# k-sheridan/mantis

Hardware: AMD Instinct MI355X
Metric: poses/sec + p50 per-frame latency, 1280x720 4-cam batch (higher is better)
Workload: dtype f64; 1 GPU; config3: 4-cam 1280x720 rig, shared map, full mantis3 path per camera + joint rig Gauss-Newton; cams_per_rig=4, contexts_per_gpu=6, landmarks=720, parallelism=rig-data-parallel x1

## Files before the change

### mantis_amd/csrc/api.hip

```cpp
#include <hip/hip_runtime.h>
#ifndef MK_FC_THREADS
#define MK_FC_THREADS 256
#endif

#include <algorithm>
#include <atomic>
#include <cfloat>
#include <chrono>
#include <cmath>
#include <cstdio>
#include <cstdlib>
#include <cstring>
#include <mutex>
#include <sstream>
#include <string>
#include <thread>
#include <vector>

#include <rccl/rccl.h>

#include "kernels.hip"

using namespace mk;

// ... 865 lines not shown
    if ((st = gauss_offsets(c, n, sh)) != MANTIS_OK) return st;
    gauss.t.join();
    if ((st = run_score(c, n, ng)) != MANTIS_OK) return st;
    if ((st = results_d2h()) != MANTIS_OK) return st;
  }
  if (sh) HIP_OK(hipMemcpyAsync(c->h_sh_flags, c->d_sh_flags, sizeof(int32_t) * ng, hipMemcpyDeviceToHost, c->s));
  HIP_OK(wait_stream(c, n));
  finish_profile(c);
  const int per = c->cfg.particles * c->cfg.iterations * 6;
  int used = 0;
  if (sh)
    for (int f = 0; f < ng; f++) used += c->h_sh_flags[f] ? 1 : 0;
  for (int f = 0; f < n; f++) {
    if (!sh && c->h_st[f].reaches_pf) used++;
    if (c->h_st[f].overflow) {
      std::ostringstream os;
      os << "frame " << f << ": workspace capacity exceeded (flags " << c->h_st[f].overflow << ", borders "
         << c->h_st[f].n_borders << ", points " << c->h_st[f].n_points << ", raw quads " << c->h_st[f].n_raw_quads
         << ")";
      c->err = os.str();
      c->h_res[f].status = MANTIS_ERR_CAPACITY;
    }
  }
  if (const char* fs = getenv("MANTIS_FRAME_STATS")) {
    if (FILE* fp = fopen(fs, "a")) {
      for (int f = 0; f < n; f++)
        fprintf(fp, "%d %d %d %d %d %d %d\n", c->h_st[f].n_runs, c->h_st[f].n_borders, c->h_st[f].n_points,
                c->h_st[f].trace_steps_max, c->h_st[f].trace_steps_sum, c->h_st[f].n_chunks, c->h_st[f].trace_ticks);
      fclose(fp);
    }
  }
  if (used * per != *c->h_gtotal) { c->err = "internal: gaussian stream accounting mismatch"; return MANTIS_ERR_DEVICE; }
  c->frame_rng.resize(n);
  if (sh) {
    std::vector<int> upto(ng + 1, 0);
    for (int f = 0; f < ng; f++) upto[f + 1] = upto[f] + (c->h_sh_flags[f] ? 1 : 0);
    for (int f = 0; f < n; f++) c->frame_rng[f] = c->h_states[upto[sh->gidx[f] + 1]];
  } else {
    int k = 0;
    for (int f = 0; f < n; f++) {
      if (c->h_st[f].reaches_pf) k++;
      c->frame_rng[f] = c->h_states[k];
    }
  }
  c->rng_state = c->h_states[used];
  return MANTIS_OK;
}

template <class T>
mantis_status dalloc(Ctx* c, T** p, size_t count) {
  if (hipMalloc((void**)p, sizeof(T) * std::max<size_t>(count, 1)) != hipSuccess) {
    c->err = "hipMalloc failed";
    return MANTIS_ERR_OOM;
  }
  return MANTIS_OK;
}
struct DevScratch {
  Ctx* c;
  std::vector<void*> p;
  explicit DevScratch(Ctx* ctx) : c(ctx) {}
  template <class T>
  bool get(T** q, size_t count) {
    *q = nullptr;
    if (dalloc(c, q, count)) return true;
    p.push_back((void*)*q);
    return false;
  }
  ~DevScratch() {
    if (!p.empty()) (void)hipStreamSynchronize(c->s);
    for (void* q : p) (void)hipFree(q);
  }
};
template <class T>
mantis_status halloc(Ctx* c, T** p, size_t count) {
  if (hipHostMalloc((void**)p, sizeof(T) * std::max<size_t>(count, 1), hipHostMallocDefault) != hipSuccess) {
    c->err = "hipHostMalloc failed";
    return MANTIS_ERR_OOM;
  }
  return MANTIS_OK;
}

std::vector<double> gather_tbc(const mantis_image* cams, int n) {
  std::vector<double> T(16 * (size_t)n);
  for (int i = 0; i < n; i++) std::memcpy(&T[16 * (size_t)i], cams[i].T_base_cam, sizeof(double) * 16);
  return T;
}

thread_local std::string g_create_err;

}

extern "C" {

int32_t mantis_abi_version(void) { return MANTIS_ABI_VERSION; }

void mantis_default_config(mantis_config* cfg) {
  std::memset(cfg, 0, sizeof(*cfg));
  cfg->struct_size = sizeof(mantis_config);
  cfg->device = 0;
  cfg->max_cams = 16;
  cfg->max_width = 1280;
  cfg->max_height = 720;
  cfg->rng_seed = 1;
  cfg->canny_low = 50;
  cfg->polygon_epsilon = 10;
  cfg->search_radius_multiplier = 0.1;
  cfg->grid_spacing = 0.32;
  cfg->particles = 50;
  cfg->iterations = 10;
  cfg->gn_enable = 0;
  cfg->gn_iterations = 10;
  cfg->max_quads = kMaxQuads;
  cfg->max_contour_points = 262144;
  cfg->quad_gn_iterations = 0;
  cfg->rig_weighting = 0;
}

mantis_status mantis_create(const mantis_config* cfg_in, void** out_ctx) {
  if (!out_ctx) return MANTIS_ERR_ARG;
  *out_ctx = nullptr;
  mantis_config cfg;
  mantis_default_config(&cfg);
  if (cfg_in) {
    if (cfg_in->struct_size != (int32_t)sizeof(mantis_config)) {
      g_create_err = "mantis_config.struct_size mismatch";
      return MANTIS_ERR_ARG;
    }
    cfg = *cfg_in;
  }
  if (cfg.max_quads == 0) cfg.max_quads = kMaxQuads;
  if ((int64_t)cfg.particles * cfg.iterations * 6 * (cfg.max_cams > 0 ? cfg.max_cams : 1) > INT32_MAX) {
    g_create_err = "particles x iterations x 6 x max_cams exceeds 2^31 gaussians per batch";
    return MANTIS_ERR_ARG;
  }
  if (cfg.particles < 1 || cfg.particles > 96 || cfg.iterations < 0 || cfg.iterations > 1000 || cfg.max_cams < 1 ||
      cfg.max_width < 3 || cfg.max_height < 3 || cfg.gn_iterations < 0 || cfg.gn_iterations > 10 ||
      cfg.quad_gn_iterations < 0 || cfg.quad_gn_iterations > 20 || cfg.rig_weighting < 0 || cfg.rig_weighting > 1) {
    g_create_err = "invalid config (particles 1..96, iterations 0..1000, gn_iterations 0..10, "
                   "quad_gn_iterations 0..20, max_cams >= 1, image >= 3x3)";
    return MANTIS_ERR_ARG;
  }
  if (cfg.max_width > 8190) {
    g_create_err = "max_width: at most 8190 (the hysteresis bands hold a row's worst-case runs in LDS)";
    return MANTIS_ERR_ARG;
  }
  if (cfg.max_height > 65533) {
    g_create_err = "max_height: at most 65533 (border walks and contour points pack y + 1 in 16 bits)";
    return MANTIS_ERR_ARG;
  }
  if ((int64_t)((cfg.max_height + HB_ROWS - 1) / HB_ROWS) * HB_ROWS * ((cfg.max_width + 1) / 2) >= (1 << 24)) {
    g_create_err = "max_width x max_height: at most 2^25 pixels (hysteresis run ids and their band row share a word)";
    return MANTIS_ERR_ARG;
  }
  if (cfg.max_quads != kMaxQuads) {
    g_create_err = "max_quads: the per-frame quad capacity is fixed at 256 in this build";
    return MANTIS_ERR_ARG;
  }
  int ndev = 0;
  if (hipGetDeviceCount(&ndev) != hipSuccess || ndev <= cfg.device) {
    g_create_err = "no HIP device available (libmantis_amd requires an MI355X / gfx950 GPU)";
    return MANTIS_ERR_DEVICE;
  }
  Ctx* c = new Ctx();
  c->cfg = cfg;
  c->rng_state = cfg.rng_seed ? cfg.rng_seed : 0xffffffffULL;
  if (hipSetDevice(cfg.device) != hipSuccess || hipStreamCreateWithFlags(&c->s, hipStreamNonBlocking) != hipSuccess ||
      hipStreamCreateWithFlags(&c->s_copy, hipStreamNonBlocking) != hipSuccess ||
      hipEventCreateWithFlags(&c->ev_gauss, hipEventDisableTiming) != hipSuccess ||
      hipEventCreateWithFlags(&c->ev_wait, hipEventDisableTiming | hipEventBlockingSync) != hipSuccess) {
    g_create_err = "hipSetDevice/hipStreamCreate failed";
    if (c->s) (void)hipStreamDestroy(c->s);
    if (c->s_copy) (void)hipStreamDestroy(c->s_copy);
    delete c;
    return MANTIS_ERR_DEVICE;
  }
  if (hipDeviceGetAttribute(&c->n_cu, hipDeviceAttributeMultiprocessorCount, cfg.device) != hipSuccess || c->n_cu < 1)
    c->n_cu = 256;
  if (const char* e = std::getenv("MANTIS_RPP_BLOCKS")) c->rpp_blocks = std::atoi(e);
  if (const char* e = std::getenv("MANTIS_OP_ROUNDS")) c->op_rounds = std::max(1, std::min(kOpMaxRounds, std::atoi(e)));
  if (const char* e = std::getenv("MANTIS_OP_SPILL")) c->op_spill = std::max(0, std::min(64, std::atoi(e)));
  if (const char* e = std::getenv("MANTIS_OP_LANES_SMALL")) c->op_lanes_small = std::max(1, std::min(64, std::atoi(e)));
  if (const char* e = std::getenv("MANTIS_OP_ROUNDS_SMALL")) c->op_rounds_small = std::max(1, std::min(kOpMaxRounds, std::atoi(e)));
  if (const char* e = std::getenv("MANTIS_SEG_M")) c->seg_m = std::max(0, std::min(4096, std::atoi(e)));
  if (const char* e = std::getenv("MANTIS_CANNY_STRIP")) c->canny_strip = c->canny_small = std::atoi(e);
  if (const char* e = std::getenv("MANTIS_CANNY_CAT")) c->canny_cat = e[0] != '0';
  if (const char* e = std::getenv("MANTIS_GN_FUSED")) c->gn_fused_all = e[0] != '0';
  if (const char* e = std::getenv("MANTIS_PF_INIT")) c->pf_init = std::max(0, std::min(2, std::atoi(e)));
  if (const char* e = std::getenv("MANTIS_HYST_REC")) c->hyst_rec = e[0] != '0';
  {
    const char* pc = std::getenv("DEBUG_CLR_GRAPH_PACKET_CAPTURE");
    c->use_graphs = pc && pc[0] == '0';
    if (const char* e = std::getenv("MANTIS_GRAPHS")) c->use_graphs = c->use_graphs && e[0] != '0';
  }
  if (const char* e = std::getenv("MANTIS_HYST_EPOCH0")) c->hyst_epoch = std::max(3, std::min(255, std::atoi(e)));
  c->F = cfg.max_cams;
  c->Wmax = cfg.max_width;
  c->Hmax = cfg.max_height;
  c->plane = (size_t)(c->Wmax + 2) * (c->Hmax + 2);
  c->bstride = bits::tiled_words(c->Wmax, c->Hmax);
  c->dstride = (size_t)dbits_wpw(c->Wmax + 2) * (c->Hmax + 2);
  c->pool_cap = cfg.max_contour_points;
  {
    c->trace_lds_max = 160 * 1024 - 512 * 8 - 64;
    c->trace_lds_ok = hipFuncSetAttribute((const void*)k_trace_borders_lds, hipFuncAttributeMaxDynamicSharedMemorySize,
                                          (int)c->trace_lds_max) == hipSuccess;
    const char* so = getenv("MANTIS_SCREEN");
    c->screen_off = so && so[0] == '0';
    const char* e = getenv("MANTIS_TRACE_LDS_FRAMES");
    c->trace_lds_frames = e ? atoi(e) : c->n_cu / 4;
    const char* e2 = getenv("MANTIS_FC_SMALL_FRAMES");
    c->fc_small_frames = e2 ? atoi(e2) : c->n_cu / 4;
    const char* e3 = getenv("MANTIS_PF_SPLIT");
    c->pf_split = !(e3 && e3[0] == '0');
  }
  {
    const size_t ml = bits::tiled_words(c->Wmax, c->Hmax) * 4;
    hipFuncAttributes a1;
    c->pf_mask_lds = 0;
    if (!getenv("MANTIS_PF_MASK_GLOBAL") &&
        hipFuncGetAttributes(&a1, (const void*)k_score_pf<kPfThreads, kPfSplit, true>) == hipSuccess &&
        a1.sharedSizeBytes + ml <= 160 * 1024 &&
        hipFuncSetAttribute((const void*)k_score_pf<kPfThreads, kPfSplit, true>,
                            hipFuncAttributeMaxDynamicSharedMemorySize, (int)ml) == hipSuccess)
      c->pf_mask_lds = ml;
  }
  {
    hipFuncAttributes a;
    if (hipFuncGetAttributes(&a, (const void*)k_hyst_rec) == hipSuccess) {
      const size_t budget = 160 * 1024 - a.sharedSizeBytes;
      if (hipFuncSetAttribute((const void*)k_hyst_rec, hipFuncAttributeMaxDynamicSharedMemorySize, (int)budget) ==
          hipSuccess)
        c->hyst_rec_lds = budget;
    }
  }
  if (hipFuncSetAttribute((const void*)k_hyst_band, hipFuncAttributeMaxDynamicSharedMemorySize,
                          (int)(3 * sizeof(uint32_t) * HB_ROWS * bits::words(c->Wmax))) != hipSuccess) {
    g_create_err = "max_width too large for the hysteresis band kernel";
    (void)hipStreamDestroy(c->s);
    delete c;
    return MANTIS_ERR_ARG;
  }
  c->morph_bh = morph_lds(c->Wmax, MB_BH) <= 160 * 1024 ? MB_BH : MB_BH_NARROW;
  if (const char* e = getenv("MANTIS_MORPH_WALK")) {
    c->morph_walk = std::max(0, atoi(e));
    c->morph_walk_small = std::max(1, c->morph_walk);
  }
  if (const char* e = getenv("MANTIS_MORPH_WALK_SMALL")) c->morph_walk_small = std::max(1, atoi(e));
  if (morph_lds(c->Wmax, c->morph_bh) > 160 * 1024 ||
      hipFuncSetAttribute((const void*)k_morph, hipFuncAttributeMaxDynamicSharedMemorySize,
                          (int)morph_lds(c->Wmax, c->morph_bh)) !=
          hipSuccess) {
    g_create_err = "max_width too large for the morphology band kernel";
    (void)hipStreamDestroy(c->s);
    delete c;
    return MANTIS_ERR_ARG;
  }
  const int F = c->F;
  const int per = cfg.particles * cfg.iterations * 6;
  mantis_status st = MANTIS_OK;
  auto chk = [&](mantis_status s) { if (st == MANTIS_OK) st = s; };
  c->fstride = (c->plane + 3) & ~(size_t)3;
  chk(dalloc(c, &c->d_strong, (size_t)F * c->fstride));
  c->lstride = (c->plane + 1) & ~(size_t)1;
  chk(dalloc(c, &c->d_lroot, (size_t)F * c->lstride));
  chk(dalloc(c, &c->d_edge, c->plane));
  chk(dalloc(c, &c->d_det, c->plane));
  chk(dalloc(c, &c->d_eb, (size_t)F * c->bstride));
  chk(dalloc(c, &c->d_b1, (size_t)F * c->bstride));
  chk(dalloc(c, &c->d_b2, (size_t)F * c->bstride));
  chk(dalloc(c, &c->d_dbits, (size_t)F * c->dstride));
  c->tstride = tbits_words(c->Wmax + 2, c->Hmax + 2);
  chk(dalloc(c, &c->d_tbits, (size_t)F * c->tstride));
  c->rstride = (size_t)c->Hmax + 3 + (c->Hmax + HB_ROWS - 1) / HB_ROWS;
  chk(dalloc(c, &c->d_rowb, (size_t)F * c->rstride));
  chk(dalloc(c, &c->d_mask, c->plane));
  chk(dalloc(c, &c->d_mbits, (size_t)F * c->bstride));
  chk(dalloc(c, &c->d_lab, (size_t)F * c->plane));
  chk(dalloc(c, &c->d_frames, (size_t)F));
  chk(dalloc(c, &c->d_borders, (size_t)F * kMaxBorders));
  chk(dalloc(c, &c->d_bcount, (size_t)F * kMaxBorders));
  chk(dalloc(c, &c->d_boff, (size_t)F * kMaxBorders));
  chk(dalloc(c, &c->d_pool, (size_t)F * 2 * c->pool_cap));
  chk(dalloc(c, &c->d_scratch, (size_t)F * 4 * c->pool_cap));
  chk(dalloc(c, &c->d_quads, (size_t)F * kMaxQuads));
  chk(dalloc(c, &c->d_rpp, (size_t)F * kMaxQuads * 2));
  chk(dalloc(c, &c->d_items, (size_t)F * kMaxQuads * 2));
  chk(dalloc(c, &c->d_refine, (size_t)F * kMaxQuads * 2 * rpp::kCand));
  chk(dalloc(c, &c->d_jobs0, (size_t)F * kMaxQuads * 2));
  chk(dalloc(c, &c->d_jobs1, (size_t)F * kMaxQuads * 2 * rpp::kCand));
  chk(dalloc(c, &c->d_rq, 1));
  {
    const size_t blocks = c->rpp_blocks > 0 ? (size_t)c->rpp_blocks : (size_t)std::max(64, 3 * c->n_cu / 2);
    c->op_cap = (int32_t)(blocks * 256);
    for (int k = 0; k < 2; k++) {
      chk(dalloc(c, &c->d_opool[k], (size_t)kOpFields * c->op_cap));
      chk(dalloc(c, &c->d_ojob[k], (size_t)c->op_cap));
    }
    chk(dalloc(c, &c->d_octl, 2 * 2 * kOpMaxRounds));
  }
  chk(dalloc(c, &c->d_gen, (size_t)F * kMaxHyps));
  chk(dalloc(c, &c->d_hyps, (size_t)F * kMaxHyps));
  chk(dalloc(c, &c->d_st, (size_t)F));
  chk(dalloc(c, &c->d_sst, (size_t)F));
  chk(dalloc(c, &c->d_dbg, (size_t)F));
  chk(dalloc(c, &c->d_res, (size_t)F));
  chk(dalloc(c, &c->d_gauss, (size_t)F * per));
// ... 909 lines not shown
```

### mantis_amd/csrc/kernels.hip

```cpp
#include <hip/hip_runtime.h>

#include <cfloat>
#include <cstdint>
#include <type_traits>

#include "mk_bits.h"
#include "mk_contour.h"
#include "mk_gn.h"
#include "mk_math.h"
#include "mk_rpp.h"
#include "mk_shard.h"
#include "mk_sort.h"
#include "mk_track.h"
#include "mk_types.h"
#include "synth.h"

namespace mk {

#ifndef MK_DPP_SCAN
#define MK_DPP_SCAN 1
#endif
__device__ inline int wave_incl_scan(int v, int lane) {
#if MK_DPP_SCAN
  (void)lane;
// ... 1975 lines not shown
    if (best > 0) rs_s = bj;
    le_eps = best <= eps;
  }
  if (!le_eps) {
    const int sl_s = pos % count, sl_e = (rs_s + sl_s) % count;
    if (lane == 0) {
      stk[0] = sl_e; stk[1] = sl_s;
      stk[2] = sl_s; stk[3] = sl_e;
    }
    top = 2;
  } else {
    if (lane == 0) { dst[0] = spx; dst[1] = spy; }
    nc = 1;
  }
  while (top > 0) {
    top--;
    int a0 = 0, a1 = 0;
    if (lane == 0) { a0 = stk[2 * top]; a1 = stk[2 * top + 1]; }
    const int sl_s = __shfl(a0, 0), sl_e = __shfl(a1, 0);
    const int epx = PtPacked::x(src[sl_e]), epy = PtPacked::y(src[sl_e]);
    int p0 = sl_s + 1;
    if (p0 >= count) p0 = 0;
    spx = PtPacked::x(src[sl_s]);
    spy = PtPacked::y(src[sl_s]);
    if (p0 != sl_e) {
      const double dx = epx - spx, dy = epy - spy;
      int L = sl_e - p0;
      if (L < 0) L += count;
      double best = 0;
      int bt = 0x7fffffff;
      for (int t = lane; t < L; t += 64) {
        int q = p0 + t;
        if (q >= count) q -= count;
        const uint32_t v = src[q];
        const double dist = fabs((PtPacked::y(v) - spy) * dx - (PtPacked::x(v) - spx) * dy);
        if (dist > best) { best = dist; bt = t; }
      }
      wave_argmax(best, bt);
      if (best > 0) rs_s = (p0 + bt) % count;
      le_eps = best * best <= eps * (dx * dx + dy * dy);
    } else {
      le_eps = true;
    }
    if (le_eps) {
      if (lane == 0) { dst[2 * nc] = spx; dst[2 * nc + 1] = spy; }
      nc++;
      if (max_dp > 0 && nc >= max_dp) return max_dp + 1;
    } else {
      if (top + 2 > cap) return -1;
      if (lane == 0) {
        stk[2 * top] = rs_s; stk[2 * top + 1] = sl_e;
        stk[2 * top + 2] = sl_s; stk[2 * top + 3] = rs_s;
      }
      top += 2;
    }
  }
  int r = 0;
  if (lane == 0) r = approx_cleanup(dst, nc, eps, true);
  return __shfl(r, 0);
}

__device__ inline bool ccomp_before(int pa, int ha, int ka, int pb, int hb, int kb) {
  if (pa != pb) return pa > pb;
  if (ha != hb) return ha < hb;
  return ka > kb;
}

#ifndef MK_LONG_BORDER
#define MK_LONG_BORDER 128
#endif
constexpr int kLongBorder = MK_LONG_BORDER;
static_assert(kLongBorder <= 128, "k_frame_contours' length buckets (count / 4) hold counts up to 128");
constexpr int kMaxLong = 512;

struct RawQuad {
  int32_t c[8];
  int32_t parent, hole, key;
};

constexpr int kTbRows = 34;
__device__ __host__ inline int tb_groups(int Wp) { return ((Wp - 2) >> 4) + 1; }
__device__ __host__ inline size_t tbits_words(int Wp, int Hp) {
  return (size_t)tb_groups(Wp) * kTbRows * (size_t)((Hp + 31) >> 5);
}
__device__ inline uint32_t tb_off(int x, int y, int G) {
  return (uint32_t)(((y >> 5) * G + (x >> 4)) * kTbRows + (y & 31));
}
__global__ __launch_bounds__(256) void k_tile_bits(const uint32_t* __restrict__ dbits, size_t dstride,
                                                   uint32_t* __restrict__ tbits, size_t tstride, int wpw, int Wp,
                                                   int Hp) {
  extern __shared__ uint32_t tl_band[];
  const int f = blockIdx.y, ty = blockIdx.x, t = threadIdx.x;
  const uint32_t* src = dbits + (size_t)f * dstride;
  const int r0 = 32 * ty - 1;
  for (int i = t; i < kTbRows * wpw; i += 256) {
    const int e = i / wpw, r = r0 + e;
    tl_band[i] = r >= 0 && r < Hp ? src[(size_t)r * wpw + (i - e * wpw)] : 0u;
  }
  __syncthreads();
  const int G = tb_groups(Wp);
  uint32_t* dst = tbits + (size_t)f * tstride + (size_t)ty * G * kTbRows;
  for (int o = t; o < G * kTbRows; o += 256) {
    const int g = o / kTbRows, e = o - g * kTbRows;
    const int p = 16 * g - 8, w = p >> 5, sh = p & 31;
    const uint32_t lo = w >= 0 ? tl_band[e * wpw + w] : 0u, hi = w + 1 < wpw ? tl_band[e * wpw + w + 1] : 0u;
    dst[o] = (lo >> sh) | (hi << (32 - sh));
  }
}
struct BitsTiled {
  const uint32_t* __restrict__ b;
  int G;
  __device__ uint32_t operator()(int x, int y) const {
    const uint32_t* p = b + tb_off(x, y, G);
    const int sh = (x & 15) + 7;
    return nb8_from_rows((p[0] >> sh) & 7u, (p[1] >> sh) & 7u, (p[2] >> sh) & 7u);
  }
};

#ifndef MK_WALK_WINDOW
#define MK_WALK_WINDOW 1
#endif
struct Walk {
  uint32_t pos, spos, p1;
  int s, prev_s, n, steps;
  int first;
  uint32_t ck, c0, c1, c2, c3;
};
__device__ inline uint32_t wpos(int x, int y) { return (uint32_t)x | ((uint32_t)y << 16); }
__device__ inline uint32_t wdelta(int s) { return (uint32_t)(fdx(s) + (fdy(s) << 16)); }
template <class NB, class EM>
__device__ inline bool walk_start(const NB& nb, int sx, int sy, bool hole, EM& em, Walk& w) {
  const uint32_t m = nb(sx, sy);
  const int s_end0 = hole ? 0 : 4;
  int s = s_end0;
  do {
    s = (s - 1) & 7;
  } while (!((m >> s) & 1u) && s != s_end0);
  w.n = 0;
  w.steps = 0;
  if (s == s_end0) {
    em(sx - 1, sy - 1);
    w.n = 1;
    return false;
  }
  w.spos = w.pos = wpos(sx, sy);
  w.p1 = wpos(sx + fdx(s), sy + fdy(s));
  w.prev_s = s ^ 4;
  w.s = s;
  w.ck = ~0u;
  return true;
}
constexpr int kSegRows = 512;
constexpr int kSegCap = 65536;
struct SegTab {
  int32_t* rowbase;
  int32_t *border, *pos, *sdir, *next, *cnt, *off;
  int cap;
};
__device__ inline SegTab seg_tab(int32_t* sc, int pool_cap) {
  const long mc = pool_cap / kChunk;
  int32_t* base = sc + 2 * (size_t)pool_cap + 3 * (size_t)mc;
  const long avail = 4L * pool_cap - (2L * pool_cap + 3L * mc) - kSegRows;
  SegTab t;
  t.cap = (int)(avail / 6 < kSegCap ? avail / 6 : kSegCap);
  t.rowbase = base;
  int32_t* q = base + kSegRows;
  t.border = q;
  t.pos = q + t.cap;
  t.sdir = q + 2 * (size_t)t.cap;
  t.next = q + 3 * (size_t)t.cap;
  t.cnt = q + 4 * (size_t)t.cap;
  t.off = q + 5 * (size_t)t.cap;
  return t;
}
constexpr int kSegUnused = -1, kSegAlias = -2, kSegStart = -3, kSegSingle = -4;
__device__ inline int seg_id_at(int x, int y, int side, int M, const int32_t* r, const uint16_t* X,
                                const int32_t* rowbase) {
  const int j0 = r[y];
  const int j = j0 + run_at(X + j0, r[y + 1] - j0, x);
  return rowbase[y / M - 1] + 2 * ((j - j0 - 1) >> 1) + side;
}
__device__ inline bool arc_has(int s, int sn, int d) { return ((d - s - 1) & 7) < ((sn - s - 1) & 7); }
__device__ inline int first_cw(uint32_t m, int d) {
  int s = d;
  do {
    s = (s - 1) & 7;
  } while (!((m >> s) & 1u) && s != d);
  return s;
}
template <class NB>
__device__ inline void seg_begin(const NB& nb, const Border& b, int Wp, uint32_t pos, int sd, Walk& w) {
  const int sx = b.start % Wp, sy = b.start / Wp;
  const int s0 = first_cw(nb(sx, sy), b.hole ? 0 : 4);
  w.spos = wpos(sx, sy);
  w.p1 = wpos(sx + fdx(s0), sy + fdy(s0));
  w.pos = pos;
  w.s = sd;
  w.prev_s = (sd + 4) & 7;
  w.n = 0;
  w.steps = 0;
  w.first = 1;
  w.ck = ~0u;
}
template <class EM>
__device__ inline bool walk_step(const uint32_t* __restrict__ tb, int G, const uint8_t* lut, EM& em, Walk& w,
                                 int M, const int32_t* r, const uint16_t* X, const int32_t* rowbase, int& nx) {
  const int x = (int)(w.pos & 0xffffu), y = (int)(w.pos >> 16);
#if MK_WALK_WINDOW
  const uint32_t tg = (uint32_t)((y >> 5) * G + (x >> 4));
  const int yr = y & 31;
  int d = yr - (int)(w.ck & 31u);
  if ((w.ck >> 5) != tg || (unsigned)d > 1u) {
    const int s0 = fdy(w.s ^ 4) < 0 ? max(yr - 1, 0) : min(yr, 30);
    typedef unsigned int u32x4a __attribute__((ext_vector_type(4), aligned(4)));
    const u32x4a v = *(const __attribute__((address_space(1))) u32x4a*)((const char*)tb + ((tg * kTbRows + s0) << 2));
    w.c0 = v.x; w.c1 = v.y; w.c2 = v.z; w.c3 = v.w;
    w.ck = (tg << 5) | (uint32_t)s0;
    d = yr - s0;
  }
  const uint32_t va = d ? w.c1 : w.c0, vb = d ? w.c2 : w.c1, vc = d ? w.c3 : w.c2;
  const int sh = (x & 15) + 7;
  const uint32_t p9 = ((va >> sh) & 7u) | (((vb >> sh) & 7u) << 3) | (((vc >> sh) & 7u) << 6);
#else
  typedef unsigned int u32x3a __attribute__((ext_vector_type(3), aligned(4)));
  const u32x3a v = *(const __attribute__((address_space(1))) u32x3a*)((const char*)tb + (tb_off(x, y, G) << 2));
  const int sh = (x & 15) + 7;
  const uint32_t p9 = ((v.x >> sh) & 7u) | (((v.y >> sh) & 7u) << 3) | (((v.z >> sh) & 7u) << 6);
#endif
  const int s = lut[(p9 << 3) | w.s];
  if (M > 0 && !w.first && y % M == 0) {
    const bool west = arc_has(w.s, s, 4);
    if (west || arc_has(w.s, s, 0)) {
      nx = seg_id_at(x, y, west ? 0 : 1, M, r, X, rowbase);
      return false;
    }
  }
  w.first = 0;
  if (s != w.prev_s) {
    em(x - 1, y - 1);
    w.n++;
    w.prev_s = s;
  }
  const uint32_t np = w.pos + wdelta(s);
  if (np == w.spos && w.pos == w.p1) {
    nx = -1;
    return false;
  }
  w.pos = np;
  w.s = (s + 4) & 7;
  w.steps++;
  return true;
}

struct BitsRows {
  const uint32_t* b;
  int wpw;
  __device__ uint32_t row3(int x, int y) const {
    const uint32_t* p = b + (size_t)y * wpw + ((x - 1) >> 5);
    const uint64_t v = ((uint64_t)p[1] << 32) | p[0];
    return (uint32_t)(v >> ((x - 1) & 31)) & 7u;
  }
  __device__ uint32_t operator()(int x, int y) const { return nb8_from_rows(row3(x, y - 1), row3(x, y), row3(x, y + 1)); }
};
__global__ __launch_bounds__(256) void k_seg_plan(const uint32_t* __restrict__ dbits, size_t dstride,
                                                  const int32_t* __restrict__ rowb, size_t rstride,
                                                  const uint16_t* __restrict__ rx, int32_t* lab, size_t plane,
                                                  const Border* __restrict__ borders, FrameState* st,
                                                  int32_t* __restrict__ scratch, int pool_cap, int Wp, int Hp,
                                                  int border_cap, int M) {
  __shared__ int32_t rb[kSegRows + 1];
  __shared__ int32_t wsum[4];
  const int f = blockIdx.x, t = threadIdx.x, lane = t & 63, wave = t >> 6;
  const int32_t* r = rowb + (size_t)f * rstride;
  const uint16_t* X = rx + (size_t)f * plane;
  int32_t* L = lab + (size_t)f * plane;
  const int nruns = r[Hp];
  const int32_t* bidx = L + nruns;
  int nb = st[f].n_borders;
  if (nb > border_cap) nb = border_cap;
  SegTab T = seg_tab(scratch + 4 * (size_t)f * pool_cap, pool_cap);
  if (nb > T.cap) {
    if (t == 0) atomicOr(&st[f].overflow, 2);
    nb = T.cap;
  }
  const Border* bs = borders + (size_t)f * border_cap;
  const int nsr = M > 0 ? (Hp - 2) / M : 0;
  bool split = M > 0 && nsr > 0 && nsr <= kSegRows && 2 * (size_t)nruns <= plane;
  static_assert(kSegRows <= 512, "two passes of 256 sampled rows");
  int carry = 0;
  for (int pass = 0; pass < 2; pass++) {
    int v = 0;
    const int k = pass * 256 + t;
    if (split && k < nsr) {
      const int y = (k + 1) * M;
      v = 2 * ((r[y + 1] - r[y] - 1) >> 1);
    }
    const int inc = wave_incl_scan(v, lane);
    if (lane == 63) wsum[wave] = inc;
    __syncthreads();
    int o = carry;
    for (int q = 0; q < wave; q++) o += wsum[q];
    if (k < kSegRows) rb[k] = o + inc - v;
    carry += wsum[0] + wsum[1] + wsum[2] + wsum[3];
    __syncthreads();
  }
  int NC = split ? carry : 0;
  if (NC + nb > T.cap) {
    split = false;
    NC = 0;
  }
  if (t == 0) {
    st[f].seg_nc = NC;
    st[f].seg_m = split ? M : 0;
  }
  for (int k = t; k < nsr && split; k += 256) T.rowbase[k] = rb[k];
  const BitsRows nbh{dbits + (size_t)f * dstride, dbits_wpw(Wp)};
  if (split) {
    for (int k = 0; k < nsr; k++) {
      const int y = (k + 1) * M, j0 = r[y], nfg = (r[y + 1] - j0 - 1) >> 1;
      for (int i = t; i < nfg; i += 256) {
        const int g = j0 + 2 * i + 1;
        const int x0 = X[g], x1 = (int)X[g + 1] - 1;
        const int fr = uf_find_c(L, g);
        const int id = rb[k] + 2 * i;
        {
          const int bg = uf_find_c(L, g - 1);
          const int own = (bg != 0 && uf_find_c(L, bg - 1) == fr) ? bg : fr;
          const uint32_t m = nbh(x0, y);
          const int sd = first_cw(m, 4);
          T.border[id] = bidx[own];
          T.pos[id] = (int32_t)wpos(x0, y);
          T.sdir[id] = sd == 4 ? kSegSingle : sd;
          T.next[id] = -1;
          T.cnt[id] = 0;
        }
        {
          const int bg = uf_find_c(L, g + 1);
          const int own = (bg != 0 && uf_find_c(L, bg - 1) == fr) ? bg : fr;
          const uint32_t m = nbh(x1, y);
          int sd = first_cw(m, 0);
          if (sd == 0) {
            sd = kSegUnused;
          } else if (x1 == x0) {
            const int sw = first_cw(m, 4);
            const uint32_t rr = ((m | (m << 8)) >> (sw + 1)) & 0xffu;
            if (arc_has(sw, (sw + 1 + __builtin_ctz(rr)) & 7, 0)) sd = kSegUnused;
          }
          T.border[id + 1] = bidx[own];
          T.pos[id + 1] = (int32_t)wpos(x1, y);
          T.sdir[id + 1] = sd;
          T.next[id + 1] = -1;
          T.cnt[id + 1] = 0;
        }
      }
    }
  }
  __syncthreads();
  for (int b = t; b < nb; b += 256) {
    const Border bb = bs[b];
    const int sx = bb.start % Wp, sy = bb.start / Wp, id = NC + b;
    T.border[id] = b;
    T.cnt[id] = 0;
    T.pos[id] = (int32_t)wpos(sx, sy);
    if (split && sy % M == 0 && sy <= Hp - 2) {
      T.sdir[id] = kSegAlias;
      int c = seg_id_at(sx, sy, bb.hole ? 1 : 0, M, r, X, rb);
      if (T.sdir[c] == kSegUnused) c--;
      T.next[id] = c;
    } else {
      T.sdir[id] = kSegStart;
      T.next[id] = -1;
    }
  }
}

__global__ __launch_bounds__(256) void k_seg_chain(FrameState* st, int32_t* __restrict__ counts,
                                                   int32_t* __restrict__ scratch, int pool_cap, int border_cap) {
  const int f = blockIdx.x, t = threadIdx.x;
  int nb = st[f].n_borders;
  if (nb > border_cap) nb = border_cap;
  int32_t* sc = scratch + 4 * (size_t)f * pool_cap;
  SegTab T = seg_tab(sc, pool_cap);
  int32_t* cnt = counts + (size_t)f * border_cap;
  for (int b = T.cap + t; b < nb; b += 256) cnt[b] = 0;
  if (nb > T.cap) nb = T.cap;
  const int NC = st[f].seg_nc, NS = NC + nb;
  for (int b = t; b < nb; b += 256) {
    const int start = T.sdir[NC + b] == kSegAlias ? T.next[NC + b] : NC + b;
    int cur = start, acc = 0, k = 0;
    bool bad = false;
    do {
      if (++k > NS || T.border[cur] != b) {
        bad = true;
        break;
      }
      T.off[cur] = acc;
      acc += T.cnt[cur];
      cur = T.next[cur];
    } while (cur >= 0 && cur != start);
    cnt[b] = acc;
    if (bad) atomicOr(&st[f].overflow, 2);
  }
  __syncthreads();
  const int max_chunks = pool_cap / kChunk;
  int nch = st[f].n_chunks;
  if (nch > max_chunks) nch = max_chunks;
  int32_t* owner = sc + 2 * (size_t)pool_cap;
  int32_t* ordv = owner + max_chunks;
  for (int c = t; c < nch; c += 256) {
    const int sg = owner[c];
    owner[c] = T.border[sg];
    ordv[c] += T.off[sg];
  }
}

#ifndef MK_TB_WAVES
#define MK_TB_WAVES 4
#endif
__global__ __launch_bounds__(64 * MK_TB_WAVES) void k_trace_borders(const uint32_t* __restrict__ tbits, size_t tstride,
                                                      const Border* __restrict__ borders, FrameState* st,
                                                      int32_t* __restrict__ scratch, int pool_cap, int Wp,
                                                      int border_cap, const int32_t* __restrict__ rowb,
                                                      size_t rstride, const uint16_t* __restrict__ rx, size_t plane) {
  const uint64_t t_start = wall_clock64();
  __shared__ uint8_t next_lut[512 * 8];
  __shared__ int32_t next_job;
  const int f = blockIdx.x, lane = threadIdx.x & 63;
  build_next_lut(next_lut, threadIdx.x, blockDim.x);
  if (threadIdx.x == 0) next_job = 0;
  __syncthreads();
  int nb = st[f].n_borders;
  if (nb > border_cap) nb = border_cap;
  const uint32_t* B = tbits + (size_t)f * tstride;
  const int wpw = dbits_wpw(Wp);
  const Border* bs = borders + (size_t)f * border_cap;
  int32_t* sc = scratch + 4 * (size_t)f * pool_cap;
  const int max_chunks = pool_cap / kChunk;
  int32_t* chunks = sc;
  int32_t* owner = sc + 2 * (size_t)pool_cap;
  int32_t* ordv = owner + max_chunks;
  int32_t* ccount = ordv + max_chunks;
  const SegTab T = seg_tab(sc, pool_cap);
  if (nb > T.cap) nb = T.cap;
  const int NC = st[f].seg_nc, M = st[f].seg_m, NS = NC + nb;
  const int32_t* r = rowb + (size_t)f * rstride;
  const uint16_t* X = rx + (size_t)f * plane;
  const BitsTiled nbh{B, tb_groups(Wp)};
  int32_t* smax = &st[f].trace_steps_max;
  ChunkEmit em{chunks, owner, ordv, ccount, &st[f].n_chunks, max_chunks, 0, -1, 0, 0, false};
  Walk w;
  int i = -1;
  bool act = false;
  bool exhausted = NS == 0;
  const uint64_t below = (1ull << lane) - 1;
  const auto finish = [&](int nx) {
    T.cnt[i] = w.n;
    T.next[i] = nx;
    em.flush();
    if (em.ovf) atomicOr(&st[f].overflow, 2);
    atomicMax(smax, w.steps);
    atomicAdd(&st[f].trace_steps_sum, w.steps);
  };
  for (;;) {
    const uint64_t idle = __ballot(!act);
    const int nidle = __popcll(idle);
    if (!exhausted && (nidle >= 16 || nidle == 64)) {
      const int leader = __ffsll((unsigned long long)idle) - 1;
      int next = 0;
      if (lane == leader) next = atomicAdd(&next_job, nidle);
      next = __shfl(next, leader);
      if (next + nidle >= NS) exhausted = true;
      if (!act) {
        const int j = next + __popcll(idle & below);
        if (j < NS) {
          const int sd = T.sdir[j];
          if (sd != kSegUnused && sd != kSegAlias) {
            i = j;
            const Border b = bs[T.border[j]];
            em.border = j; em.cur = -1; em.k = 0; em.nch = 0; em.ovf = false;
            if (sd == kSegStart) {
              act = walk_start(nbh, b.start % Wp, b.start / Wp, b.hole != 0, em, w);
              w.first = 0;
              if (!act) finish(-1);
            } else if (sd == kSegSingle) {
              const uint32_t p = (uint32_t)T.pos[j];
              em((int)(p & 0xffffu) - 1, (int)(p >> 16) - 1);
              w.n = 1;
              w.steps = 0;
              finish(-1);
            } else {
              seg_begin(nbh, b, Wp, (uint32_t)T.pos[j], sd, w);
              act = true;
            }
          }
        }
      }
      continue;
    }
    if (nidle == 64) {
      if (exhausted) break;
      continue;
    }
    int nx = -1;
    if (act && !walk_step(nbh.b, nbh.G, next_lut, em, w, M, r, X, T.rowbase, nx)) {
      act = false;
      finish(nx);
    }
  }
  if (lane == 0) atomicMax(&st[f].trace_ticks, (int32_t)(wall_clock64() - t_start));
}

extern __shared__ uint32_t tb_lds[];
struct BitsNBLds {
  int wpw;
  __device__ uint32_t row3(int x, int y) const {
    const int o = y * wpw + ((x - 1) >> 5);
    const uint64_t v = ((uint64_t)tb_lds[o + 1] << 32) | tb_lds[o];
    return (uint32_t)(v >> ((x - 1) & 31)) & 7u;
  }
  __device__ uint32_t operator()(int x, int y) const { return nb8_from_rows(row3(x, y - 1), row3(x, y), row3(x, y + 1)); }
};
template <class NB, class EM>
__device__ inline int walk_segment_lds(const NB& nb, const uint8_t* lut, EM& em, const Border& b, int Wp,
                                       uint32_t pos, int sd, int M, const int32_t* r, const uint16_t* X,
                                       const int32_t* rowbase, int& steps) {
  Walk w;
  if (sd == kSegStart) {
    if (!walk_start(nb, b.start % Wp, b.start / Wp, b.hole != 0, em, w)) {
      steps = 0;
      return -1;
    }
    w.first = 0;
  } else {
    seg_begin(nb, b, Wp, pos, sd, w);
  }
  for (;;) {
    const int x = (int)(w.pos & 0xffffu), y = (int)(w.pos >> 16);
    const uint32_t p9 = nb.row3(x, y - 1) | (nb.row3(x, y) << 3) | (nb.row3(x, y + 1) << 6);
    const int s = lut[(p9 << 3) | w.s];
    if (M > 0 && !w.first && y % M == 0) {
      const bool west = arc_has(w.s, s, 4);
      if (west || arc_has(w.s, s, 0)) {
        steps = w.steps;
        em.n_pts = w.n;
        return seg_id_at(x, y, west ? 0 : 1, M, r, X, rowbase);
      }
    }
    w.first = 0;
    if (s != w.prev_s) {
      em(x - 1, y - 1);
      w.n++;
      w.prev_s = s;
    }
    const uint32_t np = w.pos + wdelta(s);
    if (np == w.spos && w.pos == w.p1) break;
    w.pos = np;
    w.s = (s + 4) & 7;
    w.steps++;
  }
  steps = w.steps;
  em.n_pts = w.n;
  return -1;
}
__global__ __launch_bounds__(1024) void k_trace_borders_lds(const uint32_t* __restrict__ dbits, size_t dstride,
                                                            const Border* __restrict__ borders, FrameState* st,
                                                            int32_t* __restrict__ scratch, int pool_cap, int Wp,
                                                            int Hp, int border_cap, const int32_t* __restrict__ rowb,
                                                            size_t rstride, const uint16_t* __restrict__ rx,
                                                            size_t plane) {
  __shared__ uint8_t next_lut[512 * 8];
  __shared__ int32_t next_job;
  const int f = blockIdx.x;
  build_next_lut(next_lut, threadIdx.x, blockDim.x);
  if (threadIdx.x == 0) next_job = 0;
  const int wpw = dbits_wpw(Wp);
  const uint32_t* B = dbits + (size_t)f * dstride;
  for (int k = threadIdx.x; k < wpw * Hp; k += blockDim.x) tb_lds[k] = B[k];
  __syncthreads();
  int nb = st[f].n_borders;
  if (nb > border_cap) nb = border_cap;
  const Border* bs = borders + (size_t)f * border_cap;
  int32_t* sc = scratch + 4 * (size_t)f * pool_cap;
  const int max_chunks = pool_cap / kChunk;
  int32_t* chunks = sc;
  int32_t* owner = sc + 2 * (size_t)pool_cap;
  int32_t* ordv = owner + max_chunks;
  const SegTab T = seg_tab(sc, pool_cap);
  if (nb > T.cap) nb = T.cap;
  const int NC = st[f].seg_nc, M = st[f].seg_m, NS = NC + nb;
  const int32_t* r = rowb + (size_t)f * rstride;
  const uint16_t* X = rx + (size_t)f * plane;
  const BitsNBLds nbh{wpw};
  for (;;) {
    int j = 0;
    j = atomicAdd(&next_job, 1);
    if (j >= NS) break;
    const int sd = T.sdir[j];
    if (sd == kSegUnused || sd == kSegAlias) continue;
    const Border b = bs[T.border[j]];
    ChunkEmit em{chunks, owner, ordv, ordv + max_chunks, &st[f].n_chunks, max_chunks, j, -1, 0, 0, false};
    int steps = 0, nx = -1;
    if (sd == kSegSingle) {
      const uint32_t p = (uint32_t)T.pos[j];
      em((int)(p & 0xffffu) - 1, (int)(p >> 16) - 1);
      em.n_pts = 1;
    } else {
      nx = walk_segment_lds(nbh, next_lut, em, b, Wp, (uint32_t)T.pos[j], sd, M, r, X, T.rowbase, steps);
    }
    T.cnt[j] = em.n_pts;
    T.next[j] = nx;
    em.flush();
    if (em.ovf) atomicOr(&st[f].overflow, 2);
    atomicMax(&st[f].trace_steps_max, steps);
  }
}

#ifndef MK_FC_CPL
#define MK_FC_CPL 2
#endif
#ifndef MK_FC_CU
#define MK_FC_CU 8
#endif
#ifndef MK_FC_WPE
#define MK_FC_WPE 5
#endif
__global__ __launch_bounds__(1024) __attribute__((amdgpu_waves_per_eu(MK_FC_WPE))) void k_frame_contours(const uint32_t* __restrict__ dbits, size_t dstride,
                                                         const Border* __restrict__ borders,
                                                         FrameState* st, int32_t* __restrict__ counts,
                                                         int32_t* __restrict__ offs, int32_t* __restrict__ pool,
                                                         int32_t* __restrict__ scratch, int pool_cap,
                                                         QuadRec* __restrict__ quads, FrameDebug* dbg,
                                                         const FrameDesc* __restrict__ frames, int Wp, int Hp,
                                                         size_t plane, int border_cap, double eps, double search_mult,
                                                         const int32_t* __restrict__ rowb, size_t rstride,
                                                         const uint16_t* __restrict__ rx) {
  __shared__ int32_t scan[1024];
  __shared__ RawQuad raw[kMaxQuads];
  __shared__ int32_t nraw, total, nkeep;
  __shared__ int32_t idx4[kMaxQuads][4];
  __shared__ int32_t nbr[kMaxQuads];
  __shared__ int32_t kpos[kMaxQuads];
  __shared__ int32_t ord[kMaxQuads];
  __shared__ float qcx[kMaxQuads], qcy[kMaxQuads];
  __shared__ double qside[kMaxQuads];
  __shared__ int32_t nchunk, nlong;
  __shared__ int32_t longs[kMaxLong];
  const int f = blockIdx.x;
  const int tid = threadIdx.x;
  const uint32_t* B = dbits + (size_t)f * dstride;
  const int wpw = dbits_wpw(Wp);
  const Border* bs = borders + (size_t)f * border_cap;
  int32_t* cnt = counts + (size_t)f * border_cap;
  int32_t* off = offs + (size_t)f * border_cap;
  uint32_t* pl = (uint32_t*)(pool + 2 * (size_t)f * pool_cap);
  int32_t* sc = scratch + 4 * (size_t)f * pool_cap;
  int nb = st[f].n_borders;
  if (nb > border_cap) nb = border_cap;
  auto emit_raw = [&](int i, const int32_t* q4) {
    const int q = atomicAdd(&nraw, 1);
    if (q < kMaxQuads) {
      for (int k = 0; k < 8; k++) raw[q].c[k] = q4[k];
      int par = bs[i].parent;
      if (par < 0) {
        const int pr = -par - 1;
        par = run_at_row(rowb + (size_t)f * rstride, Hp, pr) * Wp + rx[(size_t)f * plane + pr];
      }
      raw[q].parent = par;
      raw[q].hole = bs[i].hole;
      raw[q].key = bs[i].key;
    } else {
      atomicOr(&st[f].overflow, 4);
    }
  };
  const uint64_t t0 = wall_clock64();
#ifdef MK_HYST_TICKS
#define MK_TICK(k)
#else
#define MK_TICK(k) \
  if (tid == 0) st[f].ticks[k] = (int32_t)(wall_clock64() - t0);
#endif
  if (tid == 0) { nraw = 0; total = 0; nlong = 0; nchunk = st[f].n_chunks; }
  __syncthreads();

  const int max_chunks = pool_cap / kChunk;
  int32_t* chunks = sc;
  int32_t* owner = sc + 2 * (size_t)pool_cap;
  int32_t* ordv = owner + max_chunks;

  {
    const int lane = tid & 63, wv = tid >> 6, nwv = blockDim.x >> 6;
    int run = 0;
    for (int base = 0; base < nb; base += blockDim.x) {
      const int i = base + tid;
      const int v = i < nb ? cnt[i] : 0;
      const int inc = wave_incl_scan(v, lane);
      if (lane == 63) scan[wv] = inc;
      __syncthreads();
      int pre = 0, tot = 0;
      for (int k = 0; k < nwv; k++) {
        const int s = scan[k];
        pre += k < wv ? s : 0;
        tot += s;
      }
      if (i < nb) off[i] = run + pre + inc - v;
      run += tot;
      __syncthreads();
    }
    if (tid == 0) total = run;
    __syncthreads();
  }
  if (total > pool_cap || nchunk > max_chunks) {
    if (tid == 0) {
      atomicOr(&st[f].overflow, 2);
      st[f].n_points = total;
      st[f].n_quads = 0;
      st[f].n_raw_quads = 0;
    }
    return;
  }
  MK_TICK(0);
  if (nchunk > 0) {
    constexpr int kCPL = MK_FC_CPL, LPC = kChunk / kCPL, CPW = 64 / LPC, kCU = MK_FC_CU;
    static_assert(kCPL == 1 || kCPL == 2, "points per lane");
    const int wave = tid >> 6, lane = tid & 63, nwaves = blockDim.x >> 6;
    const int32_t* ccount = ordv + max_chunks;
    const int l = (lane % LPC) * kCPL;
    const uint32_t* ch = (const uint32_t*)chunks;
    typedef __attribute__((aligned(8))) uint2 u2a;
    for (int c0 = wave * CPW * kCU; c0 < nchunk; c0 += nwaves * CPW * kCU) {
      int cc[kCU], b[kCU], k[kCU], o[kCU];
      uint32_t v[kCU][kCPL];
#pragma unroll
      for (int u = 0; u < kCU; u++) {
        const int c = min(c0 + u * CPW + lane / LPC, nchunk - 1);
        cc[u] = c0 + u * CPW + lane / LPC < nchunk ? ccount[c] : 0;
        b[u] = owner[c];
        k[u] = ordv[c] + l;
        if (kCPL == 2) {
          const uint2 w = *(const u2a*)(ch + (size_t)c * kChunk + l);
          v[u][0] = w.x;
          v[u][kCPL - 1] = w.y;
        } else {
          v[u][0] = ch[(size_t)c * kChunk + l];
        }
      }
#pragma unroll
      for (int u = 0; u < kCU; u++) o[u] = off[b[u]];
#pragma unroll
      for (int u = 0; u < kCU; u++)
#pragma unroll
        for (int e = 0; e < kCPL; e++)
          if (l + e < cc[u]) pl[(size_t)o[u] + k[u] + e] = v[u][e];
    }
  }
  __syncthreads();
  MK_TICK(1);
  __shared__ int32_t hist[33], nshort, next_long, next_short;
  __shared__ int32_t wstk[16][2 * kWaveStk];
  if (tid < 33) hist[tid] = 0;
  if (tid == 0) { next_long = 0; next_short = 0; }
  __syncthreads();
  bool sorted = nb <= 1024;
  if (sorted) {
    for (int i = tid; i < nb; i += blockDim.x) {
      const int c = cnt[i];
      if (c > kLongBorder) {
        const int k = atomicAdd(&nlong, 1);
        if (k < kMaxLong) longs[k] = i;
      } else {
        atomicAdd(&hist[c >> 2], 1);
      }
    }
    __syncthreads();
    sorted = nlong <= kMaxLong;
    if (sorted) {
      if (tid == 0) {
        int acc = 0;
        for (int b = 32; b >= 0; b--) {
          const int h = hist[b];
          hist[b] = acc;
          acc += h;
        }
        nshort = acc;
      }
      __syncthreads();
      for (int i = tid; i < nb; i += blockDim.x) {
        const int c = cnt[i];
        if (c <= kLongBorder) scan[atomicAdd(&hist[c >> 2], 1)] = i;
      }
      __syncthreads();
      const int lane = tid & 63;
      for (;;) {
        int k = 0;
        if (lane == 0) k = atomicAdd(&next_long, 1);
        k = __shfl(k, 0);
        if (k >= nlong) break;
        const int i = longs[k], o = off[i], c = cnt[i];
        int32_t* dst = sc + 4 * (size_t)o;
        int32_t* stk = dst + 2 * (size_t)c;
        int m = approx_poly_wave(pl + o, c, eps, dst, (lds_i32*)wstk[tid >> 6], 10, kWaveStk);
        if (m < 0) m = approx_poly_wave(pl + o, c, eps, dst, stk, 10);
        if (m == 4 && lane == 0) emit_raw(i, dst);
      }
#ifdef MK_FC_TICK_SPLIT
      MK_TICK(2);
#endif
      for (;;) {
        int k = 0;
        if (lane == 0) k = atomicAdd(&next_short, 64);
        k = __shfl(k, 0);
        if (k >= nshort) break;
        if (k + lane < nshort) {
          const int i = scan[k + lane], o = off[i], c = cnt[i];
          int32_t* dst = sc + 4 * (size_t)o;
          int32_t* stk = dst + 2 * (size_t)c;
          const int m = approx_poly(PtPacked{pl + o}, c, eps, true, dst, stk, 10);
          if (m == 4) emit_raw(i, dst);
        }
      }
      __syncthreads();
#ifdef MK_FC_TICK_SPLIT
      MK_TICK(3);
#else
      MK_TICK(2);
#endif
    } else {
      __syncthreads();
      if (tid == 0) nlong = 0;
// ... 2065 lines not shown
```

Before: 30520 rig poses/s.

## Defer border-walk segment finalization and batch chunk counter atomics in LDS

In the border-tracing kernels, segment completion (seg_id_at lookup, counts, flush, step statistics) is deferred until a refill point, so a lane that finishes does less divergent work inside the per-step loop. The row-sampling modulo becomes a reciprocal-multiply (or mask for powers of two) test. The chunk counter now lives in shared memory and is written to global memory once per block, and step max/sum are reduced per wave instead of using per-walk global atomics. This adds a pending-state variable and a minimum contour-point check, plus optional tick instrumentation.

```diff
diff --git a/mantis_amd/csrc/api.hip b/mantis_amd/csrc/api.hip
--- a/mantis_amd/csrc/api.hip
+++ b/mantis_amd/csrc/api.hip
@@ -1041,6 +1041,10 @@
     g_create_err = "max_width x max_height: at most 2^25 pixels (hysteresis run ids and their band row share a word)";
     return MANTIS_ERR_ARG;
   }
+  if (cfg.max_contour_points < kMinContourPoints) {
+    g_create_err = "max_contour_points: at least 4096 (the border walks' chunk planes and segment table share the pool's scratch)";
+    return MANTIS_ERR_ARG;
+  }
   if (cfg.max_quads != kMaxQuads) {
     g_create_err = "max_quads: the per-frame quad capacity is fixed at 256 in this build";
     return MANTIS_ERR_ARG;
diff --git a/mantis_amd/csrc/kernels.hip b/mantis_amd/csrc/kernels.hip
--- a/mantis_amd/csrc/kernels.hip
+++ b/mantis_amd/csrc/kernels.hip
@@ -2151,6 +2151,7 @@
 }
 constexpr int kSegRows = 512;
 constexpr int kSegCap = 65536;
+constexpr int kMinContourPoints = 4096;
 struct SegTab {
   int32_t* rowbase;
   int32_t *border, *pos, *sdir, *next, *cnt, *off;
@@ -2201,9 +2202,18 @@
   w.first = 1;
   w.ck = ~0u;
 }
+struct RowSample {
+  uint32_t M, inv;
+  __device__ explicit RowSample(int m)
+      : M((uint32_t)m), inv(m <= 0 || (m & (m - 1)) == 0 ? 0u : 0xffffffffu / (uint32_t)m + 1) {}
+  __device__ bool operator()(uint32_t y) const {
+    if (inv == 0) return (y & (M - 1)) == 0;
+    return y - __umulhi(y, inv) * M == 0;
+  }
+};
 template <class EM>
 __device__ inline bool walk_step(const uint32_t* __restrict__ tb, int G, const uint8_t* lut, EM& em, Walk& w,
-                                 int M, const int32_t* r, const uint16_t* X, const int32_t* rowbase, int& nx) {
+                                 int M, const RowSample& sampled, int& nx) {
   const int x = (int)(w.pos & 0xffffu), y = (int)(w.pos >> 16);
 #if MK_WALK_WINDOW
   const uint32_t tg = (uint32_t)((y >> 5) * G + (x >> 4));
@@ -2227,10 +2237,10 @@
   const uint32_t p9 = ((v.x >> sh) & 7u) | (((v.y >> sh) & 7u) << 3) | (((v.z >> sh) & 7u) << 6);
 #endif
   const int s = lut[(p9 << 3) | w.s];
-  if (M > 0 && !w.first && y % M == 0) {
+  if (M > 0 && !w.first && sampled((uint32_t)y)) {
     const bool west = arc_has(w.s, s, 4);
     if (west || arc_has(w.s, s, 0)) {
-      nx = seg_id_at(x, y, west ? 0 : 1, M, r, X, rowbase);
+      nx = west ? 0 : 1;
       return false;
     }
   }
@@ -2416,6 +2426,9 @@
 #ifndef MK_TB_WAVES
 #define MK_TB_WAVES 4
 #endif
+#ifndef MK_TB_REFILL
+#define MK_TB_REFILL 16
+#endif
 __global__ __launch_bounds__(64 * MK_TB_WAVES) void k_trace_borders(const uint32_t* __restrict__ tbits, size_t tstride,
                                                       const Border* __restrict__ borders, FrameState* st,
                                                       int32_t* __restrict__ scratch, int pool_cap, int Wp,
@@ -2423,10 +2436,10 @@
                                                       size_t rstride, const uint16_t* __restrict__ rx, size_t plane) {
   const uint64_t t_start = wall_clock64();
   __shared__ uint8_t next_lut[512 * 8];
-  __shared__ int32_t next_job;
+  __shared__ int32_t next_job, n_chunks;
   const int f = blockIdx.x, lane = threadIdx.x & 63;
   build_next_lut(next_lut, threadIdx.x, blockDim.x);
-  if (threadIdx.x == 0) next_job = 0;
+  if (threadIdx.x == 0) next_job = n_chunks = 0;
   __syncthreads();
   int nb = st[f].n_borders;
   if (nb > border_cap) nb = border_cap;
@@ -2445,25 +2458,44 @@
   const int32_t* r = rowb + (size_t)f * rstride;
   const uint16_t* X = rx + (size_t)f * plane;
   const BitsTiled nbh{B, tb_groups(Wp)};
-  int32_t* smax = &st[f].trace_steps_max;
-  ChunkEmit em{chunks, owner, ordv, ccount, &st[f].n_chunks, max_chunks, 0, -1, 0, 0, false};
+  const RowSample sampled(M);
+  ChunkEmit em{chunks, owner, ordv, ccount, &n_chunks, max_chunks, 0, -1, 0, 0, false};
   Walk w;
   int i = -1;
   bool act = false;
+  int pend = 0;
+  int steps_max = 0, steps_sum = 0;
   bool exhausted = NS == 0;
   const uint64_t below = (1ull << lane) - 1;
-  const auto finish = [&](int nx) {
-    T.cnt[i] = w.n;
-    T.next[i] = nx;
-    em.flush();
-    if (em.ovf) atomicOr(&st[f].overflow, 2);
-    atomicMax(smax, w.steps);
-    atomicAdd(&st[f].trace_steps_sum, w.steps);
+#ifdef MK_TB_TICK_SPLIT
+  int32_t tka[6] = {0, 0, 0, 0, 0, 0};
+  uint64_t tkp = wall_clock64(), tk_exh = 0;
+  const auto tick = [&](int k) {
+    const uint64_t nw = wall_clock64();
+    tka[k] += MK_TB_TICK_SPLIT == 2 ? 1 : (int32_t)(nw - tkp);
+    tkp = nw;
   };
+#endif
   for (;;) {
     const uint64_t idle = __ballot(!act);
     const int nidle = __popcll(idle);
-    if (!exhausted && (nidle >= 16 || nidle == 64)) {
+    const bool refill = !exhausted && (nidle >= MK_TB_REFILL || nidle == 64);
+    if (refill || nidle == 64) {
+      if (pend) {
+        int nx = -1;
+        if (pend > 1) nx = seg_id_at((int)(w.pos & 0xffffu), (int)(w.pos >> 16), pend - 2, M, r, X, T.rowbase);
+        T.cnt[i] = w.n;
+        T.next[i] = nx;
+        em.flush();
+        if (em.ovf) atomicOr(&st[f].overflow, 2);
+        steps_max = max(steps_max, w.steps);
+        steps_sum += w.steps;
+        pend = 0;
+      }
+#ifdef MK_TB_TICK_SPLIT
+      tick(2);
+#endif
+      if (!refill) break;
       const int leader = __ffsll((unsigned long long)idle) - 1;
       int next = 0;
       if (lane == leader) next = atomicAdd(&next_job, nidle);
@@ -2480,13 +2512,13 @@
             if (sd == kSegStart) {
               act = walk_start(nbh, b.start % Wp, b.start / Wp, b.hole != 0, em, w);
               w.first = 0;
-              if (!act) finish(-1);
+              if (!act) pend = 1;
             } else if (sd == kSegSingle) {
               const uint32_t p = (uint32_t)T.pos[j];
               em((int)(p & 0xffffu) - 1, (int)(p >> 16) - 1);
               w.n = 1;
               w.steps = 0;
-              finish(-1);
+              pend = 1;
             } else {
               seg_begin(nbh, b, Wp, (uint32_t)T.pos[j], sd, w);
               act = true;
@@ -2494,18 +2526,41 @@
           }
         }
       }
+#ifdef MK_TB_TICK_SPLIT
+      tick(3);
+      if (exhausted && !tk_exh) tk_exh = tkp;
+#endif
       continue;
     }
-    if (nidle == 64) {
-      if (exhausted) break;
-      continue;
-    }
+#ifdef MK_TB_TICK_SPLIT
+    const int nch0 = em.nch;
+#endif
     int nx = -1;
-    if (act && !walk_step(nbh.b, nbh.G, next_lut, em, w, M, r, X, T.rowbase, nx)) {
+    if (act && !walk_step(nbh.b, nbh.G, next_lut, em, w, M, sampled, nx)) {
       act = false;
-      finish(nx);
-    }
-  }
+      pend = nx + 2;
+    }
+#ifdef MK_TB_TICK_SPLIT
+    tick(__ballot(em.nch != nch0) ? 1 : 0);
+#endif
+  }
+  for (int o = 32; o > 0; o >>= 1) steps_max = max(steps_max, __shfl_xor(steps_max, o));
+  steps_sum = wave_sum(steps_sum);
+  if (lane == 0) {
+    atomicMax(&st[f].trace_steps_max, steps_max);
+    atomicAdd(&st[f].trace_steps_sum, steps_sum);
+  }
+  __syncthreads();
+  if (threadIdx.x == 0) st[f].n_chunks = n_chunks;
+#ifdef MK_TB_TICK_SPLIT
+  if (lane == 0) {
+    if (MK_TB_TICK_SPLIT != 2) {
+      tka[4] = tk_exh ? (int32_t)(tkp - tk_exh) : 0;
+      tka[5] = (int32_t)(tkp - t_start);
+    }
+    for (int k = 0; k < 6; k++) atomicAdd(&st[f].ticks[k], tka[k]);
+  }
+#endif
   if (lane == 0) atomicMax(&st[f].trace_ticks, (int32_t)(wall_clock64() - t_start));
 }
 
@@ -2568,10 +2623,10 @@
                                                             size_t rstride, const uint16_t* __restrict__ rx,
                                                             size_t plane) {
   __shared__ uint8_t next_lut[512 * 8];
-  __shared__ int32_t next_job;
+  __shared__ int32_t next_job, n_chunks;
   const int f = blockIdx.x;
   build_next_lut(next_lut, threadIdx.x, blockDim.x);
-  if (threadIdx.x == 0) next_job = 0;
+  if (threadIdx.x == 0) next_job = n_chunks = 0;
   const int wpw = dbits_wpw(Wp);
   const uint32_t* B = dbits + (size_t)f * dstride;
   for (int k = threadIdx.x; k < wpw * Hp; k += blockDim.x) tb_lds[k] = B[k];
@@ -2597,7 +2652,7 @@
     const int sd = T.sdir[j];
     if (sd == kSegUnused || sd == kSegAlias) continue;
     const Border b = bs[T.border[j]];
-    ChunkEmit em{chunks, owner, ordv, ordv + max_chunks, &st[f].n_chunks, max_chunks, j, -1, 0, 0, false};
+    ChunkEmit em{chunks, owner, ordv, ordv + max_chunks, &n_chunks, max_chunks, j, -1, 0, 0, false};
     int steps = 0, nx = -1;
     if (sd == kSegSingle) {
       const uint32_t p = (uint32_t)T.pos[j];
@@ -2612,6 +2667,8 @@
     if (em.ovf) atomicOr(&st[f].overflow, 2);
     atomicMax(&st[f].trace_steps_max, steps);
   }
+  __syncthreads();
+  if (threadIdx.x == 0) st[f].n_chunks = n_chunks;
 }
 
 #ifndef MK_FC_CPL
@@ -2672,7 +2729,7 @@
     }
   };
   const uint64_t t0 = wall_clock64();
-#ifdef MK_HYST_TICKS
+#if defined(MK_HYST_TICKS) || defined(MK_TB_TICK_SPLIT)
 #define MK_TICK(k)
 #else
 #define MK_TICK(k) \
```

Result: faster. 31090 rig poses/s (median of 6 runs) (+1.9%).
